# ytinyui/music2midi

Measured on AMD Instinct MI355X. Metric: decoded MIDI tokens/sec/node on 10 s clips, higher is better.
Workload: dtype bf16; 1 GPU; BASELINE configs[2]: full generate (log-mel + encoder + KV-cached greedy decode), bf16, batch 32 clips/GPU x 220500 samples, S=864, max_length 1024; global_batch=32, clips_per_gpu=32, rows_with_eos=0, parallelism=clip-sharded x1, weight_broadcast_bytes=0, world=1, backend=none

## Files before the change

music2midi_amd/csrc/decode.hip:

```cpp
#include "mma.h"
#include "t5.h"

#include <stdlib.h>
#include <type_traits>

namespace m2m {

#ifdef M2M_STAMPS
__device__ unsigned long long g_stamps[1 << 18];
__device__ unsigned int g_stamp_n;
#define M2M_STAMP(kid, phase)                                                                   \
  do {                                                                                          \
    if (threadIdx.x == 0 && blockIdx.x == 0 && blockIdx.y == 0) {                               \
      static_assert((phase) < 8, "phase");                                                      \
      if ((phase) == 0) m2m_stamp_base = atomicAdd(&g_stamp_n, 8u);                             \
      const unsigned long long tk = __builtin_amdgcn_s_memrealtime();                           \
      if (m2m_stamp_base + 8 <= (1u << 18))                                                     \
        g_stamps[m2m_stamp_base + (phase)] = ((unsigned long long)(kid) << 56) | ((unsigned long long)(phase) << 48) | (tk & 0xFFFFFFFFFFFFull); \
    }                                                                                           \
  } while (0)
#define M2M_STAMP_DECL unsigned int m2m_stamp_base = 0; (void)m2m_stamp_base;
#else
#define M2M_STAMP(kid, phase) do {} while (0)
#define M2M_STAMP_DECL
// ... 171 lines not shown
    if (ocol == 0 && ob < a.B) atomicMax(a.keys + ob, key);
    if (blockIdx.x == 0 && blockIdx.y == 0 && tid == 0) a.state->t = t_cur + 1;
    M2M_STAMP(2, 2);
  } else {
    if (done || tid >= 256 || ob >= a.B || on >= a.N) return;
    const int idx = orow * 17 + ocol;
    float v = red[0][idx];
    for (int w = 1; w < nw; ++w) v += red[w][idx];
    a.out[(int64_t)ob * a.ldo + on] = v;
    M2M_STAMP(2, 2);
  }
}

static bool dec_gemm_shape(int K, int* ns, int* nw) {
  switch (K) {
    case 128: *ns = 1; *nw = 4; return true;
    case 256: *ns = 2; *nw = 4; return true;
    case 384: *ns = 2; *nw = 6; return true;
    case 512: *ns = 2; *nw = 8; return true;
    default: return false;
  }
}

template <typename T>
static int launch_dec_gemm_t(const DecGemmArgs& a, hipStream_t st) {
  int ns = 0, nw = 0;
  if (!dec_gemm_shape(a.K, &ns, &nw)) {
    set_error("dec_gemm: K=%d not supported by the decode projections (128/256/384/512)", a.K);
    return M2M_ERR_INVALID;
  }
  dim3 grid((unsigned)ceil_div(a.N, 16), (unsigned)ceil_div(a.B, 16));
  dim3 block((unsigned)(64 * nw));
  if (a.keys) {
    if (ns == 1) hipLaunchKernelGGL((dec_gemm_kernel<T, 1, true>), grid, block, 0, st, a);
    else hipLaunchKernelGGL((dec_gemm_kernel<T, 2, true>), grid, block, 0, st, a);
  } else {
    if (ns == 1) hipLaunchKernelGGL((dec_gemm_kernel<T, 1, false>), grid, block, 0, st, a);
    else hipLaunchKernelGGL((dec_gemm_kernel<T, 2, false>), grid, block, 0, st, a);
  }
  M2M_CHECK_HIP(hipGetLastError());
  return M2M_OK;
}

static int launch_dec_gemm(int precision, const DecGemmArgs& a, hipStream_t st) {
  return precision == M2M_PREC_BF16 ? launch_dec_gemm_t<bf16_t>(a, st) : launch_dec_gemm_t<float>(a, st);
}

struct DecFfArgs {
  const xq_t* x;
  xq_t* x_out;
  xq_t* x_zero;
  const float* ln_w;
  float eps;
  const void* Wi;
  const void* Wo;
  int d, d_ff, B;
  DecState* state;
  int check_done;
};

constexpr int FF_C = 32;
constexpr int FF_HP = FF_C + 8;

#ifndef M2M_FF_ABL
#define M2M_FF_ABL 0
#endif
template <int FF_R>
__device__ __forceinline__ void dec_ff_carry(const DecFfArgs& a, int b0, int done) {
  const int tid = threadIdx.x, K = a.d;
  xq_t v[FF_R];
#pragma unroll
  for (int i = 0; i < FF_R; ++i) v[i] = a.x[(int64_t)min(b0 + i, a.B - 1) * K + tid];
  if (done) return;
  if (a.check_done && b0 == 0 && tid == 0) {
    if (a.state->n_unfinished == 0) { a.state->done = 1; a.state->out_len = a.state->t + 1; }
    a.state->n_unfinished = 0;
  }
#pragma unroll
  for (int i = 0; i < FF_R; ++i) {
    if (b0 + i < a.B) {
      const int64_t at = (int64_t)(b0 + i) * K + tid;
      atomicAdd(reinterpret_cast<unsigned long long*>(a.x_out + at), (unsigned long long)v[i]);
      a.x_zero[at] = 0;
    }
  }
}

#ifndef M2M_FF_MULTI_SETS
#define M2M_FF_MULTI_SETS 1
#endif
template <typename T, int KS, int FF_R, int NSL>
__device__ __forceinline__ void dec_ff_body(const DecFfArgs& a) {
  static_assert(NSL == 1 || FF_R == 8, "several slices per workgroup: the lane pairing of the 8-row form");
  M2M_STAMP_DECL
  constexpr int CPR = 32 * KS;
  __shared__ float ss_s[KS][16];
  __shared__ float red[KS][4][16 * 17];
  __shared__ __align__(16) T hs[16 * FF_HP];
  if constexpr (NSL == 1) M2M_STAMP(4, 0);
  const int done = chain_done(a.state);
  const int tid = threadIdx.x, lane = tid & 63, ks = tid >> 6;
  const int r = lane & 15, g = lane >> 4;
  const int nrb = (a.B + FF_R - 1) / FF_R, ngr = a.d_ff / (FF_C * NSL) + 1;
  const int xcd = blockIdx.x & 7, slot = blockIdx.x >> 3;
  const int c = xcd + 8 * (slot / nrb), b0 = (slot - (slot / nrb) * nrb) * FF_R;
  const int K = a.d;
  if (c >= ngr) return;
  if (c == ngr - 1) {
    dec_ff_carry<FF_R>(a, b0, done);
    return;
  }
  const int kbeg = ks * 64 + 8 * g;
  const bool row_ok = r < FF_R && (b0 + r) < a.B;
  const T* Wi = reinterpret_cast<const T*>(a.Wi);
  const T* Wo = reinterpret_cast<const T*>(a.Wo);
  const int s0 = c * NSL;

  xq2_t xraw[2][4];
  const int srow = tid >= CPR ? 1 : 0, scc = tid - srow * CPR;
  xq2_t xst[FF_R / 2];
  xq2_t* xs = nullptr;
  if constexpr (NSL == 1) {
    __shared__ __align__(16) xq2_t xs_lds[FF_R * CPR];
    xs = xs_lds;
#pragma unroll
    for (int i = 0; i < FF_R / 2; ++i)
      xst[i] = (M2M_FF_ABL & 2) ? xq2_t{1 << 28, 1 << 27} : *reinterpret_cast<const xq2_t*>(a.x + (int64_t)min(b0 + 2 * i + srow, a.B - 1) * K + 2 * scc);
    __builtin_amdgcn_sched_barrier(0);
  } else {
    const xq_t* xr = a.x + (int64_t)(b0 + (row_ok ? r : 0)) * K + kbeg;
#pragma unroll
    for (int s = 0; s < 2; ++s)
#pragma unroll
      for (int q = 0; q < 4; ++q) xraw[s][q] = (M2M_FF_ABL & 2) ? xq2_t{1 << 28, 1 << 27} : *reinterpret_cast<const xq2_t*>(xr + 32 * s + 2 * q);
  }
  float4 g0[2], g1[2];
#pragma unroll
  for (int s = 0; s < 2; ++s) {
    g0[s] = *reinterpret_cast<const float4*>(a.ln_w + kbeg + 32 * s);
    g1[s] = *reinterpret_cast<const float4*>(a.ln_w + kbeg + 32 * s + 4);
  }
  constexpr int NB = (NSL > 1 && sizeof(T) == 2) ? M2M_FF_MULTI_SETS : 1;
  Frag<T> wf[NB][4][2];
  Frag<T> wo[NB][4];
#pragma unroll
  for (int b = 0; b < NB; ++b) {
#pragma unroll
    for (int j = 0; j < 4; ++j)
#pragma unroll
      for (int s = 0; s < 2; ++s) wf[b][j][s] = load_frag(Wi + (int64_t)(2 * FF_C * (s0 + b) + 16 * j + r) * K + kbeg + 32 * s);
#pragma unroll
    for (int j = 0; j < 4; ++j) wo[b][j] = load_frag(Wo + (int64_t)(16 * (4 * ks + j) + r) * a.d_ff + FF_C * (s0 + b) + 8 * g);
  }
  __builtin_amdgcn_sched_barrier(0);
  asm volatile("" ::"s"(done));
  if constexpr (NSL == 1) {
#pragma unroll
    for (int i = 0; i < FF_R / 2; ++i) xs[row_stage_at(2 * i + srow, scc, CPR)] = xst[i];
    __syncthreads();
    const int lr = r & (FF_R - 1), lcc = (kbeg >> 1) ^ (r >= FF_R ? 4 : 0);
#pragma unroll
    for (int s = 0; s < 2; ++s)
#pragma unroll
      for (int q = 0; q < 4; ++q) xraw[s][q] = xs[row_stage_at(lr, lcc + 16 * s + q, CPR)];
  }
  float4 x0[2], x1[2];
#pragma unroll
  for (int s = 0; s < 2; ++s) {
    x0[s] = make_float4(xq_flt(xraw[s][0].x), xq_flt(xraw[s][0].y), xq_flt(xraw[s][1].x), xq_flt(xraw[s][1].y));
    x1[s] = make_float4(xq_flt(xraw[s][2].x), xq_flt(xraw[s][2].y), xq_flt(xraw[s][3].x), xq_flt(xraw[s][3].y));
  }

  float ss = 0.f;
#pragma unroll
  for (int s = 0; s < 2; ++s)
    ss += x0[s].x * x0[s].x + x0[s].y * x0[s].y + x0[s].z * x0[s].z + x0[s].w * x0[s].w +
          x1[s].x * x1[s].x + x1[s].y * x1[s].y + x1[s].z * x1[s].z + x1[s].w * x1[s].w;
  ss += lane_xor<16>(ss);
  ss += lane_xor<32>(ss);
  if (g == 0) ss_s[ks][r] = ss;
  __syncthreads();
  if constexpr (NSL == 1) M2M_STAMP(4, 3);
  float tot = 0.f;
#pragma unroll
  for (int w = 0; w < KS; ++w) tot += ss_s[w][r];
  const float rs = row_ok ? rsqrtf(tot / (float)K + a.eps) : 0.f;
  Frag<T> fa[2];
#pragma unroll
  for (int s = 0; s < 2; ++s) {
    const float xv[8] = {g0[s].x * (x0[s].x * rs), g0[s].y * (x0[s].y * rs), g0[s].z * (x0[s].z * rs),
                         g0[s].w * (x0[s].w * rs), g1[s].x * (x1[s].x * rs), g1[s].y * (x1[s].y * rs),
                         g1[s].z * (x1[s].z * rs), g1[s].w * (x1[s].w * rs)};
    fa[s] = pack_frag<T>(xv);
  }
  const int rl = 4 * (g & 1) + 2 * (g >> 1);
  xq_t* const p0 = a.x_out + (int64_t)(b0 + rl) * K + 64 * ks + r;
  const bool ok0 = rl < FF_R && b0 + rl < a.B, ok1 = rl + 1 < FF_R && b0 + rl + 1 < a.B;
  xq_t sum0[4], sum1[4];
#pragma unroll
  for (int j = 0; j < 4; ++j) { sum0[j] = 0; sum1[j] = 0; }

#pragma unroll
  for (int i = 0; i < NSL; ++i) {
    f32x4_t acc[4];
#pragma unroll
    for (int j = 0; j < 4; ++j) acc[j] = f32x4_t{0.f, 0.f, 0.f, 0.f};
#pragma unroll
    for (int s = 0; s < 2; ++s)
#pragma unroll
      for (int j = 0; j < 4; ++j) mma32_16(acc[j], fa[s], wf[i % NB][j][s]);
    if (i + NB < NSL && !(M2M_FF_ABL & 4)) {
#pragma unroll
      for (int j = 0; j < 4; ++j)
#pragma unroll
        for (int s = 0; s < 2; ++s) wf[i % NB][j][s] = load_frag(Wi + (int64_t)(2 * FF_C * (s0 + i + NB) + 16 * j + r) * K + kbeg + 32 * s);
    }
#pragma unroll
    for (int j = 0; j < 4; ++j)
#pragma unroll
      for (int q = 0; q < 4; ++q) red[ks][j][(4 * g + q) * 17 + r] = acc[j][q];
    if constexpr (NSL == 1) M2M_STAMP(4, 1);
    __syncthreads();
    if (done) return;
    for (int idx = tid; idx < FF_R * FF_C; idx += 64 * KS) {
      const int row = idx / FF_C, cc = idx % FF_C;
      const int t = cc >> 3, q = row * 17 + (cc & 7);
      float v0 = red[0][t][q], v1 = red[0][t][q + 8];
#pragma unroll
      for (int w = 1; w < KS; ++w) { v0 += red[w][t][q]; v1 += red[w][t][q + 8]; }
      hs[row * FF_HP + cc] = from_f32<T>(gelu_new_t<T>(v0) * v1);
    }
    __syncthreads();
    if constexpr (NSL == 1) M2M_STAMP(4, 5);

    const Frag<T> fh = load_frag(hs + r * FF_HP + 8 * g);
    f32x4_t o[4];
#pragma unroll
    for (int j = 0; j < 4; ++j) {
      o[j] = f32x4_t{0.f, 0.f, 0.f, 0.f};
      mma32_16(o[j], fh, wo[i % NB][j]);
    }
    if (i + NB < NSL && !(M2M_FF_ABL & 4)) {
#pragma unroll
      for (int j = 0; j < 4; ++j) wo[i % NB][j] = load_frag(Wo + (int64_t)(16 * (4 * ks + j) + r) * a.d_ff + FF_C * (s0 + i + NB) + 8 * g);
    }
    if (NSL == 1 && (M2M_FF_ABL & 1)) return;
    if constexpr (FF_R <= 8) {
#pragma unroll
      for (int j = 0; j < 4; ++j) {
        const float x2 = lane_xor<32>(o[j][2]), x3 = lane_xor<32>(o[j][3]);
        const float v0 = g < 2 ? o[j][0] : x2, v1 = g < 2 ? o[j][1] : x3;
        if constexpr (NSL == 1) {
          if (ok0) atomicAdd(reinterpret_cast<unsigned long long*>(p0 + 16 * j), (unsigned long long)xq_fix_guarded(v0, a.state));
          if (ok1) atomicAdd(reinterpret_cast<unsigned long long*>(p0 + 16 * j + K), (unsigned long long)xq_fix_guarded(v1, a.state));
        } else {
          sum0[j] += xq_fix_guarded(v0, a.state);
          sum1[j] += xq_fix_guarded(v1, a.state);
        }
      }
    } else {
#pragma unroll
      for (int j = 0; j < 4; ++j) {
        const int col = 16 * (4 * ks + j) + r;
#pragma unroll
        for (int q = 0; q < 4; ++q) {
          const int row = b0 + 4 * g + q;
          if (4 * g + q < FF_R && row < a.B)
            atomicAdd(reinterpret_cast<unsigned long long*>(a.x_out + (int64_t)row * K + col), (unsigned long long)xq_fix_guarded(o[j][q], a.state));
        }
      }
    }
  }
  if constexpr (NSL > 1) {
    if (M2M_FF_ABL & 1) return;
#pragma unroll
    for (int j = 0; j < 4; ++j) {
      if (ok0) atomicAdd(reinterpret_cast<unsigned long long*>(p0 + 16 * j), (unsigned long long)sum0[j]);
      if (ok1) atomicAdd(reinterpret_cast<unsigned long long*>(p0 + 16 * j + K), (unsigned long long)sum1[j]);
    }
  }
  if constexpr (NSL == 1) M2M_STAMP(4, 2);
}

template <typename T, int KS, int FF_R>
__global__ __launch_bounds__(64 * KS) __attribute__((amdgpu_waves_per_eu(1, 2))) void dec_ff_kernel(DecFfArgs a) {
  dec_ff_body<T, KS, FF_R, 1>(a);
}
template <typename T, int KS, int NSL>
__global__ __launch_bounds__(64 * KS) __attribute__((amdgpu_waves_per_eu(1, 2))) void dec_ff_multi_kernel(DecFfArgs a) {
  dec_ff_body<T, KS, 8, NSL>(a);
}

template <typename T, int KS, int FF_R, int NSL>
static void launch_dec_ff_ks(const DecFfArgs& a, dim3 grid, hipStream_t st) {
  if constexpr (NSL == 1) hipLaunchKernelGGL((dec_ff_kernel<T, KS, FF_R>), grid, dim3(64 * KS), 0, st, a);
  else hipLaunchKernelGGL((dec_ff_multi_kernel<T, KS, NSL>), grid, dim3(64 * KS), 0, st, a);
}
// ... 344 lines not shown
  float eres = 0.f;
  float4 e4 = make_float4(0.f, 0.f, 0.f, 0.f);
  if constexpr (FETCH) {
    const int tok = amax_key_token(kraw, fin0, a.V, a.pad_id);
    const float* er = a.emb + (int64_t)tok * a.d;
    e4 = *reinterpret_cast<const float4*>(er + xc);
    eres = er[on_];
  }
  {
    const bool own = tid * 4 < a.d;
    if (own_wave) {
      if constexpr (FETCH) xv = e4;
      else xv = make_float4(xq_flt(xr0.x), xq_flt(xr0.y), xq_flt(xr1.x), xq_flt(xr1.y));
      float ss = own ? (xv.x * xv.x + xv.y * xv.y + xv.z * xv.z + xv.w * xv.w) : 0.f;
      ss = wave_sum(ss);
      if (lane == 0) redw[wave] = ss;
    } else if (lane == 0) {
      redw[wave] = 0.f;
    }
    __syncthreads();
    M2M_STAMP(6 + (SELF ? 1 : 0), 4);
    if (own) {
      float tot = 0.f;
#pragma unroll
      for (int wv = 0; wv < 16; ++wv) tot += redw[wv];
      const float rs = rsqrtf(tot / (float)a.d + a.eps);
      put_in<T>(hn, xc + 0, gv.x * (xv.x * rs));
      put_in<T>(hn, xc + 1, gv.y * (xv.y * rs));
      put_in<T>(hn, xc + 2, gv.z * (xv.z * rs));
      put_in<T>(hn, xc + 3, gv.w * (xv.w * rs));
    }
    __syncthreads();
    M2M_STAMP(6 + (SELF ? 1 : 0), 5);
  }

  {
    float q[1];
    da_project<T, 1, LPO>(q, w, wrow, cnt, part, hn, a.d);
#ifndef M2M_STAMPS_MERGE
    M2M_STAMP(6 + (SELF ? 1 : 0), 6);
#endif
    if (part == 0 && tid < NOUT * LPO) qs[dd] = q[0];
  }
  if (SELF) {
#pragma unroll
    for (int u = 0; u < BPT; ++u)
      if (tid + 1024 * u < a.bias_stride) biasl[tid + 1024 * u] = bv[u];
    for (int n = tid + 1024 * BPT; n < a.bias_stride; n += 1024) biasl[n] = a.bias[(int64_t)hh * a.bias_stride + n];
  }
  __syncthreads();
  M2M_STAMP(6 + (SELF ? 1 : 0), 1);

  constexpr int OCH = 32 / E;
  const T* worow = reinterpret_cast<const T*>(a.Wo) + (int64_t)on_ * a.inner + hh * DK + opart * 32;
  Vec16<T> wo[OCH];
#pragma unroll
  for (int u = 0; u < OCH; ++u) wo[u].v = *reinterpret_cast<const V16*>(worow + u * E);
  const int o2 = tid >> 3, part2 = tid & 7;
  const int which2 = 1 + (o2 >> 6), dd2 = o2 & 63;
  const T* wrow2 = reinterpret_cast<const T*>(a.Wp) + ((int64_t)which2 * a.inner + hh * DK + dd2) * a.d;
  const int cnt2 = a.d / E / LPO2;
  Vec16<T> wkv[SELF ? WMAX2 : 1];
  if (SELF) {
#pragma unroll
    for (int u = 0; u < WMAX2; ++u) wkv[u].v = *reinterpret_cast<const V16*>(wrow2 + (min(u, cnt2 - 1) * LPO2 + part2) * E);
  }

  const int n_live = row_fin ? 0 : n_prev;
  float qv[E];
#pragma unroll
  for (int e = 0; e < E; ++e) qv[e] = qs[sub * E + e];
  DaSoftmax<T> sm;
  auto round = [&](const int k0, const int u, Vec16<T>& ks, Vec16<T>& vs, const int reissue ) {
    const int key = k0 + kslot + u * KPB;
    float s = 0.f;
#pragma unroll
    for (int e = 0; e < E; ++e) s = fmaf(qv[e], ks.get(e), s);
    s = group_sum<LPR>(s);
#if M2M_DA_REQUEST_FIRST
    float vrow[E];
#pragma unroll
    for (int e = 0; e < E; ++e) vrow[e] = vs.get(e);
    if (reissue == 1 || (reissue == 2 && k0 + (u + PF) * KPB < n_live)) {
      const int64_t off = kvoff(min(key + PF * KPB, last));
      ks.v = M2M_KV_LOAD(reinterpret_cast<const V16*>(Kb + off));
      vs.v = M2M_KV_LOAD(reinterpret_cast<const V16*>(Vb + off));
    }
    if (key < n_live) {
      if (SELF) s += biasl[t - key];
      sm.visit(s, vrow);
    }
#else
    if (key < n_live) {
      float vrow[E];
#pragma unroll
      for (int e = 0; e < E; ++e) vrow[e] = vs.get(e);
      if (SELF) s += biasl[t - key];
      sm.visit(s, vrow);
    }
    if (reissue == 1 || (reissue == 2 && k0 + (u + PF) * KPB < n_live)) {
      const int64_t off = kvoff(min(key + PF * KPB, last));
      ks.v = M2M_KV_LOAD(reinterpret_cast<const V16*>(Kb + off));
      vs.v = M2M_KV_LOAD(reinterpret_cast<const V16*>(Vb + off));
    }
#endif
  };
  int k0 = 0;
  for (; k0 + (2 * PF - 1) * KPB < n_live; k0 += PF * KPB) {
#pragma unroll
    for (int u = 0; u < PF; ++u) round(k0, u, kv[u], vv[u], 1);
// ... 337 lines not shown
      else if constexpr (BEAM) nxt = rest ? cb(c + __builtin_ctz(rest) + CIF) : 0x7F000000u;
      else nxt = rest ? cbase + (unsigned)(__builtin_ctz(rest) + CIF) * clip_bytes : 0x7F000000u;
#pragma unroll
      for (int u = 0; u < PF; ++u) round(k0, u, kv[st][u], vv[st][u], 2, nxt);
    }
    if (SELF && wave == 0 && lane < LPR) {
      float s = 0.f;
#pragma unroll
      for (int e = 0; e < E; ++e) s = fmaf(qv[e], kn[c][sub * E + e], s);
      s = group_sum<LPR>(s);
      s += biasl[0];
      float vrow[E];
#pragma unroll
      for (int e = 0; e < E; ++e) vrow[e] = vn[c][sub * E + e];
      visit(s, vrow);
    }
    {
      const float mw = wave_max(m_run);
      const float scale = m2m_exp<T>(m_run - mw);
      float lsum = (sub == 0) ? l_run * scale : 0.f;
      lsum = wave_sum(lsum);
      float* gp = &redg[wave * GPW + lane / LPR][sub * E];
#pragma unroll
      for (int e = 0; e < E; e += 4)
        *reinterpret_cast<float4*>(gp + e) = make_float4(acc[e] * scale, acc[e + 1] * scale, acc[e + 2] * scale, acc[e + 3] * scale);
      if (lane == 0) { redw[wave] = mw; redl[wave] = lsum; }
      __syncthreads();
      {
        float M = redw[lane & 15];
        M = fmaxf(M, lane_xor<8>(M)); M = fmaxf(M, lane_xor<4>(M)); M = fmaxf(M, lane_xor<2>(M)); M = fmaxf(M, lane_xor<1>(M));
        const float fw = m2m_exp<T>(redw[wave] - M);
        float sw = redg[wave * GPW][lane];
#pragma unroll
        for (int j = 1; j < GPW; ++j) sw += redg[wave * GPW + j][lane];
        redo[wave][lane] = sw * fw;
        if (lane == 0) redlf[wave] = redl[wave] * fw;
      }
      __syncthreads();
      if (tid < DK) {
        float s = 0.f, L = 0.f;
#pragma unroll
        for (int wv = 0; wv < 16; ++wv) {
          s += redo[wv][tid];
          L += redlf[wv];
        }
        put_in<T>(oh[c], tid, !(L <= 0.f) ? s / L : 0.f);
      }
      __syncthreads();
    }
  }
  }

  constexpr int OCH = 32 / E;
  const T* worow = reinterpret_cast<const T*>(a.Wo) + (int64_t)on_ * a.inner + hh * DK + opart * 32;
  Vec16<T> wo[OCH];
#pragma unroll
  for (int u = 0; u < OCH; ++u) wo[u].v = *reinterpret_cast<const V16*>(worow + u * E);
#pragma unroll
  for (int c = 0; c < C; ++c) {
    const int bc = min(b0 + c, nb - 1);
    float accp = 0.f;
#pragma unroll
    for (int u = 0; u < OCH; ++u) accp = chunk_dot<T>(wo[u], oh[c], opart * OCH + u, accp);
    accp += lane_xor<1>(accp);
    if (opart == 0 && tid < 2 * a.d && !st_done && b0 + c < nb) {
      xq_t add = xq_fix_guarded(accp, a.state);
      if (hh == 0) add += xrow[c][on_];
      if (!(M2M_MC_ABL & 1) || hh == 0)
        atomicAdd(reinterpret_cast<unsigned long long*>(a.x_out + (int64_t)bc * a.d + on_), (unsigned long long)add);
      if (hh == a.H - 1) a.x_zero[(int64_t)bc * a.d + on_] = 0;
    }
  }
  if (!SELF && a.book && hh == 0 && tid == 0) {
    for (int c = 0; c < C && b0 + c < nb; ++c) {
      const int b = b0 + c;
      if (!st_done) {
        const int fin = a.finished[b];
        const int next = amax_key_token(a.keys[b], fin, a.V, a.pad_id);
        if (st_t < a.max_len) a.tokens[(int64_t)a.tok_row[b] * a.max_len + st_t] = next;
        const int nf = fin | (next == a.eos_id);
        a.finished[b] = nf;
        if (!nf) atomicAdd(&a.state->n_unfinished, 1);
        a.keys[b] = 0ull;
      }
      if (b == 0) a.state->t_copy = st_t;
    }
  }
}

template <typename F>
static void launch_dec_attn_form(bool self, bool nt, const DecAttnArgs& a, F launch) {
  constexpr std::true_type yes{};
  constexpr std::false_type no{};
  auto by_nt = [&](auto s, auto fetch, auto beam) {
    if (nt) launch(s, yes, fetch, beam);
    else launch(s, no, fetch, beam);
  };
  if (a.beam_nb > 0) {
    if (self) by_nt(yes, no, yes);
    else by_nt(no, no, yes);
  } else if (self && a.emb) {
    by_nt(yes, yes, no);
  } else if (self) {
    by_nt(yes, no, no);
  } else {
    by_nt(no, no, no);
  }
}

template <typename T>
// ... 997 lines not shown

static xq_t* xbuf(m2m_session* s, const DecView& v, int which) {
  const size_t stride = (size_t)ceil_div(s->max_batch, 32) * 32 * s->m->g.d_model;
  return reinterpret_cast<xq_t*>(s->x_dec) + (size_t)which * stride + (size_t)v.b0 * s->m->g.d_model;
}

int decode_attn_clips(const m2m_session* s, int nb) {
  if (s->sw.attn_clips > 0) return s->sw.attn_clips;
  return nb >= 48 ? 4 : (nb >= 32 ? 2 : 1);
}

int decode_ff_rows(const m2m_session* s, int nb) {
  (void)nb;
  return s->sw.ff_rows > 0 ? s->sw.ff_rows : 8;
}
int decode_ff_slices(const m2m_session* s, int nb) {
  if (s->sw.ff_slices > 0) return s->sw.ff_slices;
  return nb >= 56 ? 4 : (nb >= 32 ? 2 : 1);
}

int decode_launch_attn(m2m_session* s, const DecView& v, bool self, int layer, int self_len, hipStream_t st, bool headless, bool skip_finished) {
  const m2m_model* m = s->m;
  const m2m_t5_geometry& g = m->g;
  const size_t es = m->esize;
  const int H = g.num_heads;
  const DecLayerPacked& L = m->dec[layer];
  DecAttnArgs a{};
  const double kv_step_bytes = (double)g.num_decoder_layers * 2.0 * s->B * m->inner * ((double)s->S + s->max_dec) * (double)es;
  bool nt = kv_step_bytes > 200e6;
  if (nt && !self) {
    const double per_layer = 2.0 * s->B * m->inner * (double)s->S * (double)es;
    const int resident = s->sw.kv_resident_layers >= 0 ? s->sw.kv_resident_layers : (int)(180e6 / per_layer);
    if (layer < resident) nt = false;
  }
  int clips = decode_attn_clips(s, v.nb);
  if (self && s->sw.attn_clips_self > 0) clips = s->sw.attn_clips_self;
  a.x = xbuf(s, v, self ? 0 : 1); a.x_out = xbuf(s, v, self ? 1 : 2); a.x_zero = xbuf(s, v, self ? 2 : 0);
  a.eps = g.layer_norm_eps; a.d = g.d_model;
  a.H = H; a.inner = m->inner; a.state = v.state;
  if (skip_finished && s->sw.finished_skip) { a.fin_skip = s->finished + v.b0; a.fin_stride = 1; }
  else { a.fin_skip = &v.state->zero; a.fin_stride = 0; }
  const bool beam = (s->head_mode & HEAD_BEAM) && s->beam_nb > 0;
  if (beam) {
    a.beam_nb = s->beam_nb;
    a.anc = s->anc + (int64_t)v.b0 * s->max_dec; a.anc_par = (int64_t)s->max_batch * s->max_dec; a.anc_ld = s->max_dec;
  }
  if (headless && layer == 0) {
    a.keys = s->keys + v.b0; a.finished = s->finished + v.b0; a.tokens = s->tokens; a.tok_row = s->tok_row + v.b0;
    a.max_len = s->max_dec; a.V = g.vocab_size; a.pad_id = g.pad_token_id; a.eos_id = g.eos_token_id;
    if (self) a.emb = m->shared; else a.book = 1;
  }
  if (self) {
    const size_t off = ((size_t)layer * kv_layer_elems(s, s->max_dec) + (size_t)v.b0 * H * s->max_dec * DK) * es;
    a.ln_w = L.ln0; a.Wp = L.wqkv; a.Wo = L.wo;
    a.Kc = (unsigned char*)s->self_k + off;
    a.Vc = (unsigned char*)s->self_v + off;
    a.kv_stride = s->max_dec; a.n_keys = 0; a.self_len_override = self_len;
    a.bias = s->dec_bias_tab; a.bias_stride = s->max_dec;
    return launch_dec_attn(m->precision, true, nt, a, v.nb, clips, s->sw.mc_cif, st);
  }
  const size_t per = (size_t)s->B * H * s->S * DK;
  const size_t voff = (size_t)(beam ? v.b0 / s->beam_nb : v.b0) * H * s->S * DK;
  a.ln_w = L.ln1; a.Wp = L.wcq; a.Wo = L.wco;
  a.Kc = (unsigned char*)s->cross_kv + (((size_t)layer * 2 + 0) * per + voff) * es;
  a.Vc = (unsigned char*)s->cross_kv + (((size_t)layer * 2 + 1) * per + voff) * es;
  a.kv_stride = s->S; a.n_keys = s->S; a.self_len_override = 0; a.bias = nullptr; a.bias_stride = 0;
  return launch_dec_attn(m->precision, false, nt, a, v.nb, clips, s->sw.mc_cif, st);
}

int decode_launch_step(m2m_session* s, const DecView& v, bool forced, float* logits_out, int Ld, hipStream_t st) {
  const m2m_model* m = s->m;
  const m2m_t5_geometry& g = m->g;
  const int P = m->precision;
  xq_t* xA = xbuf(s, v, 0);
  xq_t* xB = xbuf(s, v, 1);
  xq_t* xC = xbuf(s, v, 2);
  int rc;
  const bool headless = headless_for(s, forced);
  for (int l = 0; l < g.num_decoder_layers; ++l) {
    const DecLayerPacked& L = m->dec[l];
    if ((rc = decode_launch_attn(s, v, true, l, 0, st, headless, !forced))) return rc;
    if ((rc = decode_launch_attn(s, v, false, l, 0, st, headless, !forced))) return rc;
    DecFfArgs f{};
    f.x = xC; f.x_out = xA; f.x_zero = xB; f.ln_w = L.ln2; f.eps = g.layer_norm_eps;
    f.Wi = L.wi; f.Wo = L.wo_ff; f.d = g.d_model; f.d_ff = g.d_ff; f.B = v.nb; f.state = v.state;
    f.check_done = (headless && l == 0) ? 1 : 0;
    if ((rc = launch_dec_ff(P, f, decode_ff_rows(s, v.nb), decode_ff_slices(s, v.nb), st))) return rc;
  }
  DecGemmArgs a{};
  a.eps = g.layer_norm_eps; a.B = v.nb; a.state = v.state;
  a.x = xA; a.ldx = g.d_model; a.ln_w = m->dec_final_ln; a.W = m->lm_head; a.K = g.d_model; a.N = g.vocab_size;
  a.out = s->logits + (int64_t)v.b0 * m->vocab_pad; a.ldo = m->vocab_pad;
  a.keys = headless ? s->keys + v.b0 : nullptr;
  if ((rc = launch_dec_gemm(P, a, st))) return rc;
  if (headless) return M2M_OK;
  DecHeadArgs h = head_args(s, v, forced, logits_out, Ld);
  if (!forced && (s->head_mode & HEAD_BEAM)) {
    const bool processed = s->head_mode & HEAD_PROCESSED;
    return launch_dec_beam(h, beam_args(s, v), s->beam_nb, processed ? s->proc_dev : nullptr, s->gram_dev, s->gram_state + v.b0, st);
  }
  if (!forced && s->head_mode != HEAD_GREEDY) return launch_dec_select(h, s->head_mode, s->sample_dev, s->proc_dev, s->score_dev, s->gram_dev, s->gram_state, st);
  hipLaunchKernelGGL(dec_head_kernel, dim3(1), dim3(1024), 0, st, h);
  M2M_CHECK_HIP(hipGetLastError());
  return M2M_OK;
}

}

#ifdef M2M_STAMPS
extern "C" int m2m_debug_read_stamps(unsigned long long* out_host, int max_n) {
  unsigned int n = 0;
  if (hipMemcpyFromSymbol(&n, HIP_SYMBOL(m2m::g_stamp_n), sizeof(n)) != hipSuccess) return -1;
  if ((int)n > max_n) n = (unsigned)max_n;
  if (n > (1u << 18)) n = 1u << 18;
  if (n && hipMemcpyFromSymbol(out_host, HIP_SYMBOL(m2m::g_stamps), (size_t)n * 8) != hipSuccess) return -1;
  unsigned int z = 0;
  (void)hipMemcpyToSymbol(HIP_SYMBOL(m2m::g_stamp_n), &z, sizeof(z));
  void* p = nullptr;
  if (hipGetSymbolAddress(&p, HIP_SYMBOL(m2m::g_stamps)) == hipSuccess) (void)hipMemset(p, 0, sizeof(unsigned long long) << 18);
  return (int)n;
}
#endif
```

music2midi_amd/csrc/repack.hip:

```cpp
#include "t5.h"

namespace m2m {

template <typename T>
__global__ void convert_kernel(const float* __restrict__ src, T* __restrict__ dst, int64_t n) {
  int64_t i = (int64_t)blockIdx.x * blockDim.x + threadIdx.x;
  const int64_t stride = (int64_t)gridDim.x * blockDim.x;
  for (; i < n; i += stride) dst[i] = from_f32<T>(src[i]);
}

template <typename T>
__global__ void interleave_kernel(const float* __restrict__ wi0, const float* __restrict__ wi1,
                                  T* __restrict__ dst, int dff, int d, int half) {
  const int64_t n = (int64_t)2 * dff * d;
  int64_t i = (int64_t)blockIdx.x * blockDim.x + threadIdx.x;
  const int64_t stride = (int64_t)gridDim.x * blockDim.x;
  for (; i < n; i += stride) {
    const int row = (int)(i / d), col = (int)(i - (int64_t)row * d);
    const int c = row / (2 * half), r = row - c * 2 * half;
    const float* src = (r < half) ? wi0 : wi1;
    const int srow = c * half + (r < half ? r : r - half);
    dst[i] = from_f32<T>(src[(int64_t)srow * d + col]);
  }
}

static inline int grid_for(int64_t n) {
  int64_t g = (n + 255) / 256;
  return (int)(g < 1 ? 1 : (g > 2048 ? 2048 : g));
}

int launch_convert(int precision, const float* src, void* dst, int64_t n, hipStream_t st) {
  if (precision == M2M_PREC_BF16)
    hipLaunchKernelGGL(convert_kernel<bf16_t>, dim3(grid_for(n)), dim3(256), 0, st, src, (bf16_t*)dst, n);
  else
    hipLaunchKernelGGL(convert_kernel<float>, dim3(grid_for(n)), dim3(256), 0, st, src, (float*)dst, n);
  M2M_CHECK_HIP(hipGetLastError());
  return M2M_OK;
}

int launch_interleave(int precision, const float* wi0, const float* wi1, void* dst, int dff, int d, int half,
                      hipStream_t st) {
  const int64_t n = (int64_t)2 * dff * d;
  if (precision == M2M_PREC_BF16)
    hipLaunchKernelGGL(interleave_kernel<bf16_t>, dim3(grid_for(n)), dim3(256), 0, st, wi0, wi1, (bf16_t*)dst, dff, d, half);
  else
    hipLaunchKernelGGL(interleave_kernel<float>, dim3(grid_for(n)), dim3(256), 0, st, wi0, wi1, (float*)dst, dff, d, half);
  M2M_CHECK_HIP(hipGetLastError());
  return M2M_OK;
}

__global__ __launch_bounds__(256) void checksum_kernel(const uint32_t* __restrict__ w, int64_t n, unsigned long long* __restrict__ acc) {
  __shared__ unsigned long long part[4];
  unsigned long long s = 0;
  for (int64_t i = (int64_t)blockIdx.x * blockDim.x + threadIdx.x; i < n; i += (int64_t)gridDim.x * blockDim.x)
    s += (unsigned long long)w[i] * (unsigned long long)(2 * i + 1);
  for (int o = 32; o > 0; o >>= 1) s += __shfl_xor(s, o, 64);
  if ((threadIdx.x & 63) == 0) part[threadIdx.x >> 6] = s;
  __syncthreads();
  if (threadIdx.x == 0) atomicAdd(acc, part[0] + part[1] + part[2] + part[3]);
}

int launch_checksum(const void* buf, int64_t bytes, unsigned long long* acc_dev, hipStream_t st) {
  const int64_t n = bytes / 4;
  hipLaunchKernelGGL(checksum_kernel, dim3(grid_for(n)), dim3(256), 0, st, (const uint32_t*)buf, n, acc_dev);
  M2M_CHECK_HIP(hipGetLastError());
  return M2M_OK;
}

int launch_copy_f32(const float* src, float* dst, int64_t n, hipStream_t st) {
  M2M_CHECK_HIP(hipMemcpyAsync(dst, src, (size_t)n * sizeof(float), hipMemcpyDeviceToDevice, st));
  return M2M_OK;
}

int launch_fill_zero(void* dst, int64_t bytes, hipStream_t st) {
  M2M_CHECK_HIP(hipMemsetAsync(dst, 0, (size_t)bytes, st));
  return M2M_OK;
}

}
```

music2midi_amd/csrc/t5.h:

```cpp
#pragma once

#include "common.h"
#include "env.h"

#include <vector>

namespace m2m {

constexpr int DK = 64;

struct EncLayerPacked {
  const float* ln0;
  const void* wqkv;
  const void* wo;
  const float* ln1;
  const void* wi;
  const void* wo_ff;
};

struct DecLayerPacked {
  const float* ln0;
  const void* wqkv;
  const void* wo;
  const float* ln1;
  const void* wcq;
  const void* wco;
  const float* ln2;
  const void* wi;
  const void* wo_ff;
};

}

struct m2m_model {
  m2m_t5_geometry g;
  int precision;
  int inner;
  int vocab_pad;
  size_t esize;
  void* blob = nullptr;
  int64_t blob_bytes = 0;
  std::vector<m2m::EncLayerPacked> enc;
  std::vector<m2m::DecLayerPacked> dec;
  const float* enc_final_ln = nullptr;
  const float* dec_final_ln = nullptr;
  const float* shared = nullptr;
  const void* lm_head = nullptr;
  const void* wckv = nullptr;
  std::vector<float> enc_rel_bias_host;
  std::vector<float> dec_rel_bias_host;
};

namespace m2m {

struct DecState {
  int t;
  int done;
  int out_len;
  int n_unfinished;
  int max_steps;
  int overflow;
  int t_copy;
  int zero;
  int smp_unfinished;
  int smp_ticket;
};

struct SampleParams {
  float temperature;
  int top_k;
  float top_p;
  int pad_;
  unsigned long long seed;
};

constexpr int PROC_MAX_VOCAB = 4096;
constexpr int PROC_BITS = PROC_MAX_VOCAB / 32;
constexpr int PROC_MAX_LEN = 2048;
constexpr int PROC_MAX_BAD = 64;
constexpr int PROC_MAX_BAD_IDS = 512;
struct ProcessParams {
  float penalty;
  int ngram;
// ... 173 lines not shown

namespace m2m {

enum { EPI_STORE = 0, EPI_RESID = 1, EPI_GATED = 2, EPI_HEADS = 3, EPI_STORE_F32 = 4, EPI_GATED16 = 5, EPI_GATED_TRAIN = 6, EPI_GATED_BWD = 7 };

struct GemmArgs {
  const void* A;
  const void* W;
  int M, N, K;
  void* out;
  int ldo;
  int Bsz, S, H, inner;
  int vt_which;
  void* vt_out;
  int Sp;
  int ng;
  const float* resid;
  uint32_t drop_thresh;
  float drop_scale;
  uint64_t drop_key;
  const uint64_t* drop_step;
  void* ab_out;
  const float* nx;
  const float* nw;
  float neps;
  void* h_out;
};

int launch_gemm(int precision, int epi, const GemmArgs& a, hipStream_t st);
int launch_norm_gemm(int precision, int epi, const GemmArgs& a, hipStream_t st);
bool gemm_takes_gated_train(int precision, int M, int N, int K);
bool gemm_takes_gated_bwd(int precision, int M, int N, int K);
int launch_rmsnorm(int precision, const float* x, const float* w, void* out, int M, int d, float eps, hipStream_t st);
struct AttnArgs {
  const void* Q;
  const void* K;
  const void* Vt;
  int Sp;
  const float* bias_tab;
  int tab_stride, tab_center;
  void* out;
  int B, H, Sq, Sk;
  int bias_far;
};
int launch_attn(int precision, const AttnArgs& a, bool causal, hipStream_t st);
int launch_transpose_v(int precision, const void* v, void* vt, int BH, int S, int Sp, hipStream_t st);
int launch_embed_rows(const int64_t* ids, const float* table, float* x, int M, int d, int V, int pad_id, hipStream_t st);
int launch_final_norm_f32(const float* x, const float* w, float* out_f32, void* out_T, int precision, int M, int d,
                          float eps, hipStream_t st);

int launch_convert(int precision, const float* src, void* dst, int64_t n, hipStream_t st);
int launch_interleave(int precision, const float* wi0, const float* wi1, void* dst, int dff, int d, int half,
                      hipStream_t st);
int launch_copy_f32(const float* src, float* dst, int64_t n, hipStream_t st);
int launch_fill_zero(void* dst, int64_t bytes, hipStream_t st);
int launch_checksum(const void* buf, int64_t bytes, unsigned long long* acc_dev, hipStream_t st);

int decode_init(m2m_session* s, const DecView& v, int max_steps, bool forced, hipStream_t st);
int decode_launch_step(m2m_session* s, const DecView& v, bool forced, float* logits_out, int Ld, hipStream_t st);
int decode_launch_attn(m2m_session* s, const DecView& v, bool self, int layer, int self_len, hipStream_t st, bool headless = false,
                       bool skip_finished = false);
int decode_move_rows(m2m_session* s, const int* src, const int* dst, int n, int t, hipStream_t st);
int decode_finalize(m2m_session* s, const DecView& v, hipStream_t st);
constexpr int HEAD_GREEDY = 0, HEAD_SAMPLE = 1, HEAD_BEAM = 2;
constexpr int HEAD_PROCESSED = 4;
constexpr int HEAD_SCORED = 8;
constexpr int BEAM_MAX = 32;
int decode_beam_init(m2m_session* s, const DecView& v, hipStream_t st);
int decode_beam_finalize(m2m_session* s, int rows, int steps, int64_t* out, float* scores, int max_length, hipStream_t st);
constexpr int SAMPLE_MAX_VOCAB = 4096;
int decode_attn_clips(const m2m_session* s, int nb);
int decode_ff_rows(const m2m_session* s, int nb);
int decode_ff_slices(const m2m_session* s, int nb);

}
```

music2midi_amd/csrc/t5_api.hip:

```cpp
#include "carver.h"
#include "env.h"
#include "t5.h"

#include <math.h>
#include <stdlib.h>
#include <string.h>
#include <algorithm>
#include <memory>
#include <vector>

using namespace m2m;

extern "C" int m2m_rel_bucket(int rel, int bidirectional, int num_buckets, int max_distance) {
  int bucket = 0;
  int nb = num_buckets;
  int n;
  if (bidirectional) {
    nb /= 2;
    if (rel > 0) bucket += nb;
    n = rel < 0 ? -rel : rel;
  } else {
    n = rel < 0 ? -rel : 0;
  }
  const int max_exact = nb / 2;
  if (n < max_exact) return bucket + n;
  const float ratio = logf((float)n / (float)max_exact) / (float)log((double)max_distance / (double)max_exact);
  int large = max_exact + (int)(ratio * (float)(nb - max_exact));
  if (large > nb - 1) large = nb - 1;
  return bucket + large;
}

extern "C" int m2m_model_create(const m2m_t5_geometry* geom, const m2m_t5_weights* w, int precision, void* stream,
                                m2m_model** out) {
  M2M_REQUIRE(geom && w && out, "m2m_model_create: null argument");
  M2M_REQUIRE(precision == M2M_PREC_FP32 || precision == M2M_PREC_BF16, "m2m_model_create: bad precision %d", precision);
  const m2m_t5_geometry& g = *geom;
  M2M_REQUIRE(g.d_kv == DK, "m2m_model_create: d_kv=%d unsupported (attention kernels are specialised for 64)", g.d_kv);
  M2M_REQUIRE(g.d_model == 128 || g.d_model == 256 || g.d_model == 384 || g.d_model == 512,
              "m2m_model_create: d_model=%d must be 128, 256, 384 or 512 (the reduction lengths the decode kernels are "
              "instantiated for; the fused decode attention projects with 2 lanes per output column of a 1024-thread workgroup)",
              g.d_model);
  M2M_REQUIRE(g.d_ff >= 64 && g.d_ff % 64 == 0, "m2m_model_create: d_ff=%d must be a multiple of 64", g.d_ff);
  M2M_REQUIRE((g.num_heads * g.d_kv) % 128 == 0 && g.num_heads * g.d_kv <= 1152, "m2m_model_create: num_heads*d_kv=%d must be a multiple of 128, <= 1152", g.num_heads * g.d_kv);
  M2M_REQUIRE(g.num_heads >= 1 && g.num_layers >= 1 && g.num_decoder_layers >= 1 && g.vocab_size >= 2,
              "m2m_model_create: bad geometry");
  M2M_REQUIRE(g.pad_token_id >= 0 && g.pad_token_id < g.vocab_size && g.eos_token_id >= 0 && g.eos_token_id < g.vocab_size &&
                  g.decoder_start_token_id >= 0 && g.decoder_start_token_id < g.vocab_size,
              "m2m_model_create: pad_token_id=%d, eos_token_id=%d and decoder_start_token_id=%d must lie in [0, vocab_size=%d)",
              g.pad_token_id, g.eos_token_id, g.decoder_start_token_id, g.vocab_size);
  M2M_REQUIRE(g.num_buckets >= 4 && g.num_buckets % 2 == 0 && g.max_distance > g.num_buckets / 2,
              "m2m_model_create: bad relative-attention geometry");
  M2M_REQUIRE(w->shared && w->lm_head && w->enc_rel_bias && w->dec_rel_bias && w->enc_final_ln && w->dec_final_ln &&
                  w->enc && w->dec, "m2m_model_create: null weight pointer");
  hipStream_t st = (hipStream_t)stream;
  const int d = g.d_model, dff = g.d_ff, inner = g.num_heads * g.d_kv, V = g.vocab_size;
  const int Le = g.num_layers, Ld = g.num_decoder_layers;
  const size_t es = precision == M2M_PREC_BF16 ? 2 : 4;
  const int vocab_pad = ceil_div(V, 16) * 16;

  m2m_model* m = new m2m_model();
  m->g = g; m->precision = precision; m->inner = inner; m->vocab_pad = vocab_pad; m->esize = es;
  m->enc.resize(Le); m->dec.resize(Ld);
  Carver c;
  auto F = [&](const float*& member, int64_t elems) { c.take(member, elems * 4); };
  auto T = [&](const void*& member, int64_t elems) { c.take(member, elems * es); };
  for (EncLayerPacked& L : m->enc) {
    F(L.ln0, d); T(L.wqkv, (int64_t)3 * inner * d); T(L.wo, (int64_t)d * inner);
    F(L.ln1, d); T(L.wi, (int64_t)2 * dff * d); T(L.wo_ff, (int64_t)d * dff);
  }
  for (DecLayerPacked& L : m->dec) {
    F(L.ln0, d); T(L.wqkv, (int64_t)3 * inner * d); T(L.wo, (int64_t)d * inner);
    F(L.ln1, d); T(L.wcq, (int64_t)inner * d); T(L.wco, (int64_t)d * inner);
    F(L.ln2, d); T(L.wi, (int64_t)2 * dff * d); T(L.wo_ff, (int64_t)d * dff);
  }
  F(m->enc_final_ln, d); F(m->dec_final_ln, d);
  F(m->shared, (int64_t)V * d);
  T(m->lm_head, (int64_t)vocab_pad * d);
  T(m->wckv, (int64_t)Ld * 2 * inner * d);
  m->blob_bytes = c.off;
  hipError_t e = hipMalloc(&m->blob, (size_t)c.off);
  if (e != hipSuccess) {
    set_error("m2m_model_create: hipMalloc(%lld) failed: %s", (long long)c.off, hipGetErrorString(e));
    delete m;
    return M2M_ERR_NOMEM;
  }
  c.bind((unsigned char*)m->blob);
  int rc = M2M_OK;
  if (hipMemsetAsync(m->blob, 0, (size_t)c.off, st) != hipSuccess) { set_error("m2m_model_create: hipMemsetAsync failed"); rc = M2M_ERR_HIP; }
  auto at = [&](const void* member, int64_t part = 0) { return (unsigned char*)const_cast<void*>(member) + part * inner * d * (int64_t)es; };
  auto conv = [&](const float* src, void* dst, int64_t n) {
    if (rc == M2M_OK && !src) { set_error("m2m_model_create: null layer weight pointer"); rc = M2M_ERR_INVALID; }
    if (rc == M2M_OK) rc = launch_convert(precision, src, dst, n, st);
  };
  auto copyf = [&](const float* src, const float* dst, int64_t n) {
    if (rc == M2M_OK && !src) { set_error("m2m_model_create: null layer weight pointer"); rc = M2M_ERR_INVALID; }
    if (rc == M2M_OK) rc = launch_copy_f32(src, const_cast<float*>(dst), n, st);
  };
  auto interleave = [&](const float* wi0, const float* wi1, const void* dst, int half) {
    if (rc == M2M_OK && !(wi0 && wi1)) { set_error("m2m_model_create: null wi pointer"); rc = M2M_ERR_INVALID; }
    if (rc == M2M_OK) rc = launch_interleave(precision, wi0, wi1, at(dst), dff, d, half, st);
  };
  for (int l = 0; l < Le && rc == M2M_OK; ++l) {
    const m2m_enc_layer_weights& s = w->enc[l];
    const EncLayerPacked& L = m->enc[l];
    copyf(s.ln0, L.ln0, d); copyf(s.ln1, L.ln1, d);
    conv(s.q, at(L.wqkv, 0), (int64_t)inner * d); conv(s.k, at(L.wqkv, 1), (int64_t)inner * d); conv(s.v, at(L.wqkv, 2), (int64_t)inner * d);
    conv(s.o, at(L.wo), (int64_t)d * inner);
    interleave(s.wi0, s.wi1, L.wi, 32);
    conv(s.wo, at(L.wo_ff), (int64_t)d * dff);
  }
  for (int l = 0; l < Ld && rc == M2M_OK; ++l) {
    const m2m_dec_layer_weights& s = w->dec[l];
    const DecLayerPacked& L = m->dec[l];
    copyf(s.ln0, L.ln0, d); copyf(s.ln1, L.ln1, d); copyf(s.ln2, L.ln2, d);
    conv(s.q, at(L.wqkv, 0), (int64_t)inner * d); conv(s.k, at(L.wqkv, 1), (int64_t)inner * d); conv(s.v, at(L.wqkv, 2), (int64_t)inner * d);
    conv(s.o, at(L.wo), (int64_t)d * inner);
    conv(s.cq, at(L.wcq), (int64_t)inner * d);
    conv(s.co, at(L.wco), (int64_t)d * inner);
    interleave(s.wi0, s.wi1, L.wi, 8);
    conv(s.wo, at(L.wo_ff), (int64_t)d * dff);
    conv(s.ck, at(m->wckv, l * 2 + 0), (int64_t)inner * d); conv(s.cv, at(m->wckv, l * 2 + 1), (int64_t)inner * d);
  }
  copyf(w->enc_final_ln, m->enc_final_ln, d); copyf(w->dec_final_ln, m->dec_final_ln, d);
  copyf(w->shared, m->shared, (int64_t)V * d);
  if (rc == M2M_OK) rc = launch_fill_zero(at(m->lm_head), (int64_t)vocab_pad * d * es, st);
  conv(w->lm_head, at(m->lm_head), (int64_t)V * d);
  m->enc_rel_bias_host.resize((size_t)g.num_buckets * g.num_heads);
  m->dec_rel_bias_host.resize((size_t)g.num_buckets * g.num_heads);
  hipError_t he = hipSuccess;
  if (rc == M2M_OK) he = hipMemcpyAsync(m->enc_rel_bias_host.data(), w->enc_rel_bias, m->enc_rel_bias_host.size() * 4, hipMemcpyDeviceToHost, st);
  if (rc == M2M_OK && he == hipSuccess) he = hipMemcpyAsync(m->dec_rel_bias_host.data(), w->dec_rel_bias, m->dec_rel_bias_host.size() * 4, hipMemcpyDeviceToHost, st);
  if (rc == M2M_OK && he == hipSuccess) he = hipStreamSynchronize(st);
  if (rc == M2M_OK && he != hipSuccess) { set_error("m2m_model_create: %s", hipGetErrorString(he)); rc = M2M_ERR_HIP; }
  if (rc != M2M_OK) {
    (void)hipFree(m->blob);
    delete m;
    return rc;
  }
  *out = m;
  return M2M_OK;
}

extern "C" void m2m_model_destroy(m2m_model* m) {
  if (!m) return;
  if (m->blob) (void)hipFree(m->blob);
  delete m;
}
extern "C" int m2m_model_precision(const m2m_model* m) { return m ? m->precision : M2M_ERR_INVALID; }
extern "C" int64_t m2m_model_param_bytes(const m2m_model* m) { return m ? m->blob_bytes : (int64_t)M2M_ERR_INVALID; }

extern "C" int m2m_model_checksum(const m2m_model* m, uint64_t* out_host, void* stream) {
  M2M_REQUIRE(m && out_host, "m2m_model_checksum: null argument");
  hipStream_t st = (hipStream_t)stream;
  unsigned long long* acc = nullptr;
  M2M_CHECK_HIP(hipMalloc((void**)&acc, sizeof(unsigned long long)));
  unsigned long long host = 0;
  hipError_t e = hipMemsetAsync(acc, 0, sizeof(unsigned long long), st);
  int rc = M2M_OK;
  if (e == hipSuccess) rc = launch_checksum(m->blob, m->blob_bytes, acc, st);
  if (e == hipSuccess && rc == M2M_OK) e = hipMemcpyAsync(&host, acc, sizeof(host), hipMemcpyDeviceToHost, st);
  if (e == hipSuccess && rc == M2M_OK) e = hipStreamSynchronize(st);
  (void)hipFree(acc);
  if (rc != M2M_OK) return rc;
  if (e != hipSuccess) { set_error("m2m_model_checksum: %s", hipGetErrorString(e)); return M2M_ERR_HIP; }
  *out_host = (uint64_t)host;
  return M2M_OK;
}

namespace {
void carve_workspace(m2m_session* s, Carver& c) {
  const m2m_model* m = s->m;
  const m2m_t5_geometry& g = m->g;
  const int B = s->max_batch, S = s->max_enc, L = s->max_dec;
// ... 870 lines not shown
```

Baseline: 167,000 tokens/s.

## Pre-pack decoder FF and attention output weights into per-lane fragment images

Adds repack kernels that rearrange the decoder feed-forward Wi/Wo weights and the self- and cross-attention output projection weights into lane-ordered images at model load. The decode kernels then read each fragment as a contiguous 16-byte-per-lane block instead of strided row gathers, so weight loads coalesce. The cost is extra device memory for the duplicated images and more load-time work.

```diff
diff --git a/music2midi_amd/csrc/decode.hip b/music2midi_amd/csrc/decode.hip
--- a/music2midi_amd/csrc/decode.hip
+++ b/music2midi_amd/csrc/decode.hip
@@ -247,8 +247,7 @@
   xq_t* x_zero;
   const float* ln_w;
   float eps;
-  const void* Wi;
-  const void* Wo;
+  const void* Wimg;
   int d, d_ff, B;
   DecState* state;
   int check_done;
@@ -284,6 +283,13 @@
 #ifndef M2M_FF_MULTI_SETS
 #define M2M_FF_MULTI_SETS 1
 #endif
+__device__ __forceinline__ Frag<bf16_t> ff_img_frag(const bf16_t* p, int f) { return load_frag(p + f * FF_IMG_FRAG); }
+__device__ __forceinline__ Frag<float> ff_img_frag(const float* p, int f) {
+  Frag<float> v;
+  v.lo = *reinterpret_cast<const float4*>(p + f * FF_IMG_FRAG);
+  v.hi = *reinterpret_cast<const float4*>(p + f * FF_IMG_FRAG + FF_IMG_FRAG / 2);
+  return v;
+}
 template <typename T, int KS, int FF_R, int NSL>
 __device__ __forceinline__ void dec_ff_body(const DecFfArgs& a) {
   static_assert(NSL == 1 || FF_R == 8, "several slices per workgroup: the lane pairing of the 8-row form");
@@ -307,9 +313,9 @@
   }
   const int kbeg = ks * 64 + 8 * g;
   const bool row_ok = r < FF_R && (b0 + r) < a.B;
-  const T* Wi = reinterpret_cast<const T*>(a.Wi);
-  const T* Wo = reinterpret_cast<const T*>(a.Wo);
   const int s0 = c * NSL;
+  const T* const Wimg = reinterpret_cast<const T*>(a.Wimg) + (int64_t)ks * FF_IMG_WAVE + lane * (16 / (int)sizeof(T));
+  constexpr int64_t SLICE = (int64_t)KS * FF_IMG_WAVE;
 
   xq2_t xraw[2][4];
   const int srow = tid >= CPR ? 1 : 0, scc = tid - srow * CPR;
@@ -343,9 +349,9 @@
 #pragma unroll
     for (int j = 0; j < 4; ++j)
 #pragma unroll
-      for (int s = 0; s < 2; ++s) wf[b][j][s] = load_frag(Wi + (int64_t)(2 * FF_C * (s0 + b) + 16 * j + r) * K + kbeg + 32 * s);
-#pragma unroll
-    for (int j = 0; j < 4; ++j) wo[b][j] = load_frag(Wo + (int64_t)(16 * (4 * ks + j) + r) * a.d_ff + FF_C * (s0 + b) + 8 * g);
+      for (int s = 0; s < 2; ++s) wf[b][j][s] = ff_img_frag(Wimg + (s0 + b) * SLICE, 2 * j + s);
+#pragma unroll
+    for (int j = 0; j < 4; ++j) wo[b][j] = ff_img_frag(Wimg + (s0 + b) * SLICE, 8 + j);
   }
   __builtin_amdgcn_sched_barrier(0);
   asm volatile("" ::"s"(done));
@@ -408,7 +414,7 @@
 #pragma unroll
       for (int j = 0; j < 4; ++j)
 #pragma unroll
-        for (int s = 0; s < 2; ++s) wf[i % NB][j][s] = load_frag(Wi + (int64_t)(2 * FF_C * (s0 + i + NB) + 16 * j + r) * K + kbeg + 32 * s);
+        for (int s = 0; s < 2; ++s) wf[i % NB][j][s] = ff_img_frag(Wimg + (s0 + i + NB) * SLICE, 2 * j + s);
     }
 #pragma unroll
     for (int j = 0; j < 4; ++j)
@@ -437,7 +443,7 @@
     }
     if (i + NB < NSL && !(M2M_FF_ABL & 4)) {
 #pragma unroll
-      for (int j = 0; j < 4; ++j) wo[i % NB][j] = load_frag(Wo + (int64_t)(16 * (4 * ks + j) + r) * a.d_ff + FF_C * (s0 + i + NB) + 8 * g);
+      for (int j = 0; j < 4; ++j) wo[i % NB][j] = ff_img_frag(Wimg + (s0 + i + NB) * SLICE, 8 + j);
     }
     if (NSL == 1 && (M2M_FF_ABL & 1)) return;
     if constexpr (FF_R <= 8) {
@@ -888,10 +894,10 @@
   M2M_STAMP(6 + (SELF ? 1 : 0), 1);
 
   constexpr int OCH = 32 / E;
-  const T* worow = reinterpret_cast<const T*>(a.Wo) + (int64_t)on_ * a.inner + hh * DK + opart * 32;
+  const T* woimg = reinterpret_cast<const T*>(a.Wo) + ((int64_t)hh * OCH * 2 * a.d + min(tid, 2 * a.d - 1)) * E;
   Vec16<T> wo[OCH];
 #pragma unroll
-  for (int u = 0; u < OCH; ++u) wo[u].v = *reinterpret_cast<const V16*>(worow + u * E);
+  for (int u = 0; u < OCH; ++u) wo[u].v = *reinterpret_cast<const V16*>(woimg + (int64_t)u * 2 * a.d * E);
   const int o2 = tid >> 3, part2 = tid & 7;
   const int which2 = 1 + (o2 >> 6), dd2 = o2 & 63;
   const T* wrow2 = reinterpret_cast<const T*>(a.Wp) + ((int64_t)which2 * a.inner + hh * DK + dd2) * a.d;
@@ -1335,10 +1341,10 @@
   }
 
   constexpr int OCH = 32 / E;
-  const T* worow = reinterpret_cast<const T*>(a.Wo) + (int64_t)on_ * a.inner + hh * DK + opart * 32;
+  const T* woimg = reinterpret_cast<const T*>(a.Wo) + ((int64_t)hh * OCH * 2 * a.d + min(tid, 2 * a.d - 1)) * E;
   Vec16<T> wo[OCH];
 #pragma unroll
-  for (int u = 0; u < OCH; ++u) wo[u].v = *reinterpret_cast<const V16*>(worow + u * E);
+  for (int u = 0; u < OCH; ++u) wo[u].v = *reinterpret_cast<const V16*>(woimg + (int64_t)u * 2 * a.d * E);
 #pragma unroll
   for (int c = 0; c < C; ++c) {
     const int bc = min(b0 + c, nb - 1);
@@ -2442,7 +2448,7 @@
   }
   if (self) {
     const size_t off = ((size_t)layer * kv_layer_elems(s, s->max_dec) + (size_t)v.b0 * H * s->max_dec * DK) * es;
-    a.ln_w = L.ln0; a.Wp = L.wqkv; a.Wo = L.wo;
+    a.ln_w = L.ln0; a.Wp = L.wqkv; a.Wo = L.wo_img;
     a.Kc = (unsigned char*)s->self_k + off;
     a.Vc = (unsigned char*)s->self_v + off;
     a.kv_stride = s->max_dec; a.n_keys = 0; a.self_len_override = self_len;
@@ -2451,7 +2457,7 @@
   }
   const size_t per = (size_t)s->B * H * s->S * DK;
   const size_t voff = (size_t)(beam ? v.b0 / s->beam_nb : v.b0) * H * s->S * DK;
-  a.ln_w = L.ln1; a.Wp = L.wcq; a.Wo = L.wco;
+  a.ln_w = L.ln1; a.Wp = L.wcq; a.Wo = L.wco_img;
   a.Kc = (unsigned char*)s->cross_kv + (((size_t)layer * 2 + 0) * per + voff) * es;
   a.Vc = (unsigned char*)s->cross_kv + (((size_t)layer * 2 + 1) * per + voff) * es;
   a.kv_stride = s->S; a.n_keys = s->S; a.self_len_override = 0; a.bias = nullptr; a.bias_stride = 0;
@@ -2473,7 +2479,7 @@
     if ((rc = decode_launch_attn(s, v, false, l, 0, st, headless, !forced))) return rc;
     DecFfArgs f{};
     f.x = xC; f.x_out = xA; f.x_zero = xB; f.ln_w = L.ln2; f.eps = g.layer_norm_eps;
-    f.Wi = L.wi; f.Wo = L.wo_ff; f.d = g.d_model; f.d_ff = g.d_ff; f.B = v.nb; f.state = v.state;
+    f.Wimg = L.ff_img; f.d = g.d_model; f.d_ff = g.d_ff; f.B = v.nb; f.state = v.state;
     f.check_done = (headless && l == 0) ? 1 : 0;
     if ((rc = launch_dec_ff(P, f, decode_ff_rows(s, v.nb), decode_ff_slices(s, v.nb), st))) return rc;
   }
diff --git a/music2midi_amd/csrc/repack.hip b/music2midi_amd/csrc/repack.hip
--- a/music2midi_amd/csrc/repack.hip
+++ b/music2midi_amd/csrc/repack.hip
@@ -49,6 +49,55 @@
   return M2M_OK;
 }
 
+template <typename T>
+__global__ void ff_image_kernel(const T* __restrict__ wi, const T* __restrict__ wo, T* __restrict__ img, int dff, int d) {
+  constexpr int EPC = 16 / (int)sizeof(T), HPF = 8 / EPC;
+  const int KS = d / 64;
+  const int64_t n = (int64_t)3 * dff * d / EPC;
+  const int64_t stride = (int64_t)gridDim.x * blockDim.x;
+  for (int64_t i = (int64_t)blockIdx.x * blockDim.x + threadIdx.x; i < n; i += stride) {
+    const int lane = (int)(i & 63), r = lane & 15, g = lane >> 4;
+    int64_t q = i >> 6;
+    const int half = (int)(q % HPF); q /= HPF;
+    const int f = (int)(q % 12); q /= 12;
+    const int ks = (int)(q % KS), c = (int)(q / KS);
+    const T* src = f < 8 ? wi + (int64_t)(64 * c + 16 * (f >> 1) + r) * d + 64 * ks + 32 * (f & 1) + 8 * g
+                         : wo + (int64_t)(16 * (4 * ks + f - 8) + r) * dff + 32 * c + 8 * g;
+    reinterpret_cast<uint4*>(img)[i] = *reinterpret_cast<const uint4*>(src + EPC * half);
+  }
+}
+
+int launch_ff_image(int precision, const void* wi, const void* wo_ff, void* img, int dff, int d, hipStream_t st) {
+  const int64_t n = (int64_t)3 * dff * d / (precision == M2M_PREC_BF16 ? 8 : 4);
+  if (precision == M2M_PREC_BF16)
+    hipLaunchKernelGGL(ff_image_kernel<bf16_t>, dim3(grid_for(n)), dim3(256), 0, st, (const bf16_t*)wi, (const bf16_t*)wo_ff, (bf16_t*)img, dff, d);
+  else
+    hipLaunchKernelGGL(ff_image_kernel<float>, dim3(grid_for(n)), dim3(256), 0, st, (const float*)wi, (const float*)wo_ff, (float*)img, dff, d);
+  M2M_CHECK_HIP(hipGetLastError());
+  return M2M_OK;
+}
+
+template <typename T>
+__global__ void attn_out_image_kernel(const T* __restrict__ wo, T* __restrict__ img, int H, int d) {
+  constexpr int E = 16 / (int)sizeof(T), OCH = 32 / E;
+  const int64_t n = (int64_t)H * OCH * 2 * d;
+  const int64_t stride = (int64_t)gridDim.x * blockDim.x;
+  for (int64_t i = (int64_t)blockIdx.x * blockDim.x + threadIdx.x; i < n; i += stride) {
+    const int tid = (int)(i % (2 * d)), u = (int)((i / (2 * d)) % OCH), h = (int)(i / ((int64_t)2 * d * OCH));
+    reinterpret_cast<uint4*>(img)[i] = *reinterpret_cast<const uint4*>(wo + (int64_t)(tid >> 1) * (H * 64) + 64 * h + 32 * (tid & 1) + E * u);
+  }
+}
+
+int launch_attn_out_image(int precision, const void* wo, void* img, int H, int d, hipStream_t st) {
+  const int64_t n = (int64_t)H * 64 * d / (precision == M2M_PREC_BF16 ? 8 : 4);
+  if (precision == M2M_PREC_BF16)
+    hipLaunchKernelGGL(attn_out_image_kernel<bf16_t>, dim3(grid_for(n)), dim3(256), 0, st, (const bf16_t*)wo, (bf16_t*)img, H, d);
+  else
+    hipLaunchKernelGGL(attn_out_image_kernel<float>, dim3(grid_for(n)), dim3(256), 0, st, (const float*)wo, (float*)img, H, d);
+  M2M_CHECK_HIP(hipGetLastError());
+  return M2M_OK;
+}
+
 __global__ __launch_bounds__(256) void checksum_kernel(const uint32_t* __restrict__ w, int64_t n, unsigned long long* __restrict__ acc) {
   __shared__ unsigned long long part[4];
   unsigned long long s = 0;
diff --git a/music2midi_amd/csrc/t5.h b/music2midi_amd/csrc/t5.h
--- a/music2midi_amd/csrc/t5.h
+++ b/music2midi_amd/csrc/t5.h
@@ -28,7 +28,13 @@
   const float* ln2;
   const void* wi;
   const void* wo_ff;
-};
+  const void* ff_img;
+  const void* wo_img;
+  const void* wco_img;
+};
+
+constexpr int FF_IMG_FRAG = 512;
+constexpr int FF_IMG_WAVE = 12 * FF_IMG_FRAG;
 
 }
 
@@ -308,6 +314,8 @@
 int launch_convert(int precision, const float* src, void* dst, int64_t n, hipStream_t st);
 int launch_interleave(int precision, const float* wi0, const float* wi1, void* dst, int dff, int d, int half,
                       hipStream_t st);
+int launch_ff_image(int precision, const void* wi, const void* wo_ff, void* img, int dff, int d, hipStream_t st);
+int launch_attn_out_image(int precision, const void* wo, void* img, int H, int d, hipStream_t st);
 int launch_copy_f32(const float* src, float* dst, int64_t n, hipStream_t st);
 int launch_fill_zero(void* dst, int64_t bytes, hipStream_t st);
 int launch_checksum(const void* buf, int64_t bytes, unsigned long long* acc_dev, hipStream_t st);
diff --git a/music2midi_amd/csrc/t5_api.hip b/music2midi_amd/csrc/t5_api.hip
--- a/music2midi_amd/csrc/t5_api.hip
+++ b/music2midi_amd/csrc/t5_api.hip
@@ -71,7 +71,8 @@
   for (DecLayerPacked& L : m->dec) {
     F(L.ln0, d); T(L.wqkv, (int64_t)3 * inner * d); T(L.wo, (int64_t)d * inner);
     F(L.ln1, d); T(L.wcq, (int64_t)inner * d); T(L.wco, (int64_t)d * inner);
-    F(L.ln2, d); T(L.wi, (int64_t)2 * dff * d); T(L.wo_ff, (int64_t)d * dff);
+    F(L.ln2, d); T(L.wi, (int64_t)2 * dff * d); T(L.wo_ff, (int64_t)d * dff); T(L.ff_img, (int64_t)3 * dff * d);
+    T(L.wo_img, (int64_t)d * inner); T(L.wco_img, (int64_t)d * inner);
   }
   F(m->enc_final_ln, d); F(m->dec_final_ln, d);
   F(m->shared, (int64_t)V * d);
@@ -117,8 +118,11 @@
     conv(s.o, at(L.wo), (int64_t)d * inner);
     conv(s.cq, at(L.wcq), (int64_t)inner * d);
     conv(s.co, at(L.wco), (int64_t)d * inner);
+    if (rc == M2M_OK) rc = launch_attn_out_image(precision, L.wo, at(L.wo_img), g.num_heads, d, st);
+    if (rc == M2M_OK) rc = launch_attn_out_image(precision, L.wco, at(L.wco_img), g.num_heads, d, st);
     interleave(s.wi0, s.wi1, L.wi, 8);
     conv(s.wo, at(L.wo_ff), (int64_t)d * dff);
+    if (rc == M2M_OK) rc = launch_ff_image(precision, L.wi, L.wo_ff, at(L.ff_img), dff, d, st);
     conv(s.ck, at(m->wckv, l * 2 + 0), (int64_t)inner * d); conv(s.cv, at(m->wckv, l * 2 + 1), (int64_t)inner * d);
   }
   copyf(w->enc_final_ln, m->enc_final_ln, d); copyf(w->dec_final_ln, m->dec_final_ln, d);
```

Measured after the change: 174,500 tokens/s (median of 6 runs). +4.5%, better.
